# lelecaruso/NavierStokes_Project_NM4PDE

Hardware: AMD Instinct MI355X
Metric: time-steps/sec (assemble_time_step + solve_time_step), 3D flow past a cylinder, P2/P1, Yosida, per-rank ILU(0) (higher is better)
Workload: dtype f64

## Files before the change

### include/nsx.h

```cpp
#ifndef NSX_H
#define NSX_H

#include <stdint.h>

#ifdef __cplusplus
extern "C" {
#endif

typedef struct nsx_handle nsx_handle;

typedef enum {
  NSX_OK = 0,
  NSX_ERR_ARG = -1,
  NSX_ERR_HIP = -2,
  NSX_ERR_UNSUPPORTED = -3,
  NSX_ERR_NOCONV = -4,
  NSX_ERR_NUMERIC = -5,
  NSX_ERR_COMM = -6
} nsx_status;

typedef enum { NSX_PREC_YOSIDA = 0, NSX_PREC_SIMPLE = 1, NSX_PREC_AYOSIDA = 2, NSX_PREC_ASIMPLE = 3 } nsx_prec;

enum {
  NSX_TEMAM = 1,
// ... 168 lines not shown

int nsx_profile_enable(nsx_handle *h, int on);
int nsx_profile_reset(nsx_handle *h);
int nsx_profile_count(nsx_handle *h);
int nsx_profile_get(nsx_handle *h, int i, const char **name, int64_t *launches, double *total_ms, double *bytes_per_launch);

int nsx_persistent_state(nsx_handle *h, int state[4]);

int nsx_path_info(nsx_handle *h, int info[32]);

#define NSX_ILU_FACTOR_LEVEL 1
#define NSX_ILU_FACTOR_LDS 2
#define NSX_ILU_FACTOR_DENSE_ROW 3
#define NSX_ILU_FACTOR_GENERAL 4
#define NSX_ILU_INVERT_NONE 0
#define NSX_ILU_INVERT_LDS 1
#define NSX_ILU_INVERT_GLOBAL 2
#define NSX_ILU_SOLVE_LEVELLED 1
#define NSX_ILU_SOLVE_DENSE 2
#define NSX_ILU_SOLVE_LANES 3
#define NSX_ILU_SOLVE_BLOCK_LDS 4
#define NSX_ILU_SOLVE_BLOCK_GLOBAL 5
int nsx_ilu_path_info(nsx_handle *h, int which, int info[16]);

int nsx_gram_schmidt_cycle(nsx_handle *h, int n, int m, double *vectors, double norm_guard, double *coeffs, double *norms2);
int nsx_gram_schmidt_sweeps(nsx_handle *h, int n, int split, int gap, int m, double *vectors, double norm_guard, int flags, double *coeffs,
                            double *norms2, double *norms2_before, int *normalized);

enum {
  NSX_BLAS1_DOT = 0, NSX_BLAS1_ADD_AND_DOT, NSX_BLAS1_ADD, NSX_BLAS1_ADD_DEV, NSX_BLAS1_SADD, NSX_BLAS1_SCALE, NSX_BLAS1_SCALE_DEV_INV,
  NSX_BLAS1_SCALE_VEC, NSX_BLAS1_AXPY_MULTI, NSX_BLAS1_AXPY_MULTI_INTO, NSX_BLAS1_CG_UPDATE, NSX_BLAS1_CG_DIRECTION, NSX_BLAS1_RECIPROCAL,
  NSX_BLAS1_FINALIZE, NSX_BLAS1_READ, NSX_BLAS1_WRITE_SCALAR, NSX_BLAS1_KIND_COUNT
};
#define NSX_BLAS1_MAX_K 40
typedef struct nsx_blas1_op {
  int32_t kind;
  int32_t d, v, w, x;
  int32_t slot, num, den;
  int32_t count;
  int32_t read;
  int32_t n;
  int32_t k;
  int32_t vs[NSX_BLAS1_MAX_K];
  double a, s;
  double coef[NSX_BLAS1_MAX_K];
} nsx_blas1_op;
// ... 22 lines not shown
```

### navierstokes_project_nm4pde_amd/csrc/nsx_blas.hip

```cpp
#include "nsx_grid.hpp"
#include "nsx_ilu_lanes.hpp"

namespace nsx {

constexpr int RED_BLOCKS = 512;
constexpr int RED_STRIDE = 1024;

struct SRef {
  double c;
  int num, den;
  int num_nb, den_nb;
};

__device__ __forceinline__ double wave_sum_all(double v) {
#pragma unroll
  for (int o = 32; o > 0; o >>= 1) v += __shfl_xor(v, o, 64);
  return v;
}

__device__ __forceinline__ double slot_value(const double *__restrict__ scal, const double *__restrict__ partial, int slot, int nb,
                                             double *sh) {
  if (nb == 0) return scal[slot];
  if (threadIdx.x < 64) {
    const double *p = partial + (size_t)slot * RED_STRIDE;
// ... 505 lines not shown
  if (!h || !info || which < 0 || which > 1) return NSX_ERR_ARG;
  for (int k = 0; k < 16; ++k) info[k] = 0;
  if (!h->have_mesh) return NSX_OK;
  const nsx::IluSchedule &s = which == 0 ? h->schedF : h->schedS;
  const bool stream = s.stream_ncomp > 0 && !s.levelled;
  info[0] = s.path.factor;
  info[1] = s.path.invert;
  info[2] = s.path.solve;
  info[3] = stream ? s.stream_epl : 0;
  info[4] = s.path.solve_pf;
  info[5] = s.path.solve_ncomp;
  info[6] = s.path.solve_f32;
  info[7] = stream ? s.n_waves : 0;
  info[8] = s.n_blocks;
  info[9] = s.max_rows;
  info[10] = s.max_block_nnz;
  info[11] = stream ? s.max_wave_rows : 0;
  info[12] = s.levelled ? 1 : 0;
  info[13] = s.packed_ok ? 1 : 0;
  info[14] = s.dense ? 1 : 0;
  info[15] = s.path.factor_lds_bytes;
  return NSX_OK;
}
```

### navierstokes_project_nm4pde_amd/csrc/nsx_ilu.hip

```cpp
#include <atomic>

#include "nsx_internal.hpp"
#include "nsx_ilu_lanes.hpp"

namespace nsx {

constexpr int ILU_WAVES = 4;
constexpr int ILU_MAXROW = 1024;

__device__ __forceinline__ void pk_store(double *__restrict__ pk_val, float *__restrict__ pk_val32, int sl, double v, int *err) {
  if (pk_val32) {
    const float f = (float)v;
    pk_val32[sl] = f;
    if (!(fabsf(f) <= 3.402823466e+38f)) __hip_atomic_store(err, 5, __ATOMIC_RELAXED, __HIP_MEMORY_SCOPE_SYSTEM);
  } else {
    pk_val[sl] = v;
  }
}

__global__ __launch_bounds__(ILU_WAVES * 64) void k_ilu_factor(const int32_t *__restrict__ bptr, const int32_t *__restrict__ lvl_off,
                                                              const int32_t *__restrict__ lvl_ptr, const int32_t *__restrict__ lvl_rows,
                                                              const int32_t *__restrict__ rp, const int32_t *__restrict__ ci,
                                                              const int32_t *__restrict__ diag, const double *__restrict__ a,
                                                              double *__restrict__ lu, const int32_t *__restrict__ slot_of,
// ... 65 lines not shown
  __shared__ int s_rp[113], s_dg[112];
  const int blk = blockIdx.x, r0 = bptr[blk], n = bptr[blk + 1] - r0;
  const int j = threadIdx.x;
  for (int t = threadIdx.x; t <= n; t += 128) s_rp[t] = rp[r0 + t];
  for (int t = threadIdx.x; t < n; t += 128) s_dg[t] = diag[r0 + t];
  __syncthreads();
  if (j < n) {
    for (int i = 0; i < n; ++i) {
      const int pe = s_dg[i];
      double acc = i == j ? 1.0 : 0.0;
      for (int p = s_rp[i]; p < pe; ++p) {
        const int k = ci[p] - r0;
        if (k >= 0) acc -= lu[p] * Ps[k * n + j];
      }
      Ps[i * n + j] = acc;
    }
    for (int i = n - 1; i >= 0; --i) {
      const int pd = s_dg[i], pe = s_rp[i + 1];
      double acc = lu[pd] * Ps[i * n + j];
      for (int p = pd + 1; p < pe; ++p) {
        const int k = ci[p] - r0;
        if (k < n) acc -= lu[p] * Ps[k * n + j];
      }
      Ps[i * n + j] = acc;
    }
  }
  __syncthreads();
  double *Pb = P + off[blk];
  for (int q = threadIdx.x; q < n * n; q += 128) Pb[q] = Ps[q];
}

__global__ __launch_bounds__(256) void k_ilu_invert(const int32_t *__restrict__ bptr, const int64_t *__restrict__ off,
                                                    const int32_t *__restrict__ rp, const int32_t *__restrict__ ci,
                                                    const int32_t *__restrict__ diag, const double *__restrict__ lu, double *P) {
  const int blk = blockIdx.x, r0 = bptr[blk], n = bptr[blk + 1] - r0;
  double *Pb = P + off[blk];
  for (int j = threadIdx.x; j < n; j += 256) {
    for (int i = 0; i < n; ++i) {
      const int row = r0 + i, pe = diag[row];
      double acc = i == j ? 1.0 : 0.0;
      for (int p = rp[row]; p < pe; ++p) {
        const int k = ci[p] - r0;
        if (k >= 0) acc -= lu[p] * Pb[(size_t)k * n + j];
      }
      Pb[(size_t)i * n + j] = acc;
    }
// ... 371 lines not shown
      s.path.factor = NSX_ILU_FACTOR_LDS;
      s.path.factor_lds_bytes = (int)lds;
      static std::atomic<size_t> lds_allowed{64 * 1024};
      if (lds > lds_allowed.load()) {
        HIP_CHECK(hipFuncSetAttribute((const void *)k_ilu_factor_lds, hipFuncAttributeMaxDynamicSharedMemorySize, 80 * 1024));
        lds_allowed.store(80 * 1024);
      }
      hipLaunchKernelGGL(k_ilu_factor_lds, dim3(s.n_blocks), dim3(ILU_WAVES * 64), lds, h->stream, s.fac_order.p, s.block_ptr.p, s.blk_lvl_off.p, s.fwd_lvl_ptr.p,
                         s.fwd_rows.p, g.rowptr.p, g.colind.p, g.diag.p, s.in_lo.p, s.in_cptr.p, s.in_cpos.p, vals, lu,
                         s.packed_ok ? s.pk_slot_of.p : nullptr, s.pk_val.p, s.pk_dinv.p, err, s.pk_dinv_slot.p, s.max_rows, (int)s.max_block_nnz, pk32);
    } else if (small_ok && s.max_rows <= ILU_DENSE_ROWS) {
      s.path.factor = NSX_ILU_FACTOR_DENSE_ROW;
      hipLaunchKernelGGL(k_ilu_factor_small, dim3(s.n_blocks), dim3(ILU_WAVES * 64), 0, h->stream, s.block_ptr.p, s.blk_lvl_off.p,
                         s.fwd_lvl_ptr.p, s.fwd_rows.p, g.rowptr.p, g.colind.p, g.diag.p, vals, lu, s.packed_ok ? s.pk_slot_of.p : nullptr,
                         s.pk_val.p, s.pk_dinv.p, err, s.pk_dinv_slot.p, pk32);
    } else {
      s.path.factor = NSX_ILU_FACTOR_GENERAL;
      hipLaunchKernelGGL(k_ilu_factor, dim3(s.n_blocks), dim3(ILU_WAVES * 64), 0, h->stream, s.block_ptr.p, s.blk_lvl_off.p, s.fwd_lvl_ptr.p,
                         s.fwd_rows.p, g.rowptr.p, g.colind.p, g.diag.p, vals, lu, s.packed_ok ? s.pk_slot_of.p : nullptr, s.pk_val.p,
                         s.pk_dinv.p, err, s.pk_dinv_slot.p, pk32);
    }
  }
  s.path.invert = NSX_ILU_INVERT_NONE;
  if (s.dense) {
    LaunchScope ls(h, "ilu_invert", 8.0 * (double)s.dn_entries + 12.0 * g.nnz());
    const bool inv_lds = env_on("NSX_ILU_INVERT_LDS");
    const size_t shm = (size_t)s.max_rows * s.max_rows * sizeof(double);
    if (inv_lds && s.max_rows <= 112) {
      static bool attr_set = false;
      if (!attr_set && shm > 64 * 1024) {
        HIP_CHECK(hipFuncSetAttribute((const void *)k_ilu_invert_lds, hipFuncAttributeMaxDynamicSharedMemorySize, 112 * 112 * (int)sizeof(double)));
        attr_set = true;
      }
      s.path.invert = NSX_ILU_INVERT_LDS;
      hipLaunchKernelGGL(k_ilu_invert_lds, dim3(s.n_blocks), dim3(128), shm, h->stream, s.block_ptr.p, s.dn_off.p, g.rowptr.p, g.colind.p, g.diag.p, lu, s.dn_P.p);
    } else {
      s.path.invert = NSX_ILU_INVERT_GLOBAL;
      hipLaunchKernelGGL(k_ilu_invert, dim3(s.n_blocks), dim3(256), 0, h->stream, s.block_ptr.p, s.dn_off.p, g.rowptr.p, g.colind.p, g.diag.p, lu,
                         s.dn_P.p);
    }
  }
}

template <int NCOMP, int LW, bool USE_LDS>
__global__ __launch_bounds__(256) void k_ilu_solve(const int32_t *__restrict__ bptr, const int32_t *__restrict__ offF,
                                                   const int32_t *__restrict__ ptrF, const int32_t *__restrict__ rowsF,
                                                   const int32_t *__restrict__ offB, const int32_t *__restrict__ ptrB,
                                                   const int32_t *__restrict__ rowsB, const int32_t *__restrict__ rp,
                                                   const int32_t *__restrict__ ci, const int32_t *__restrict__ diag,
                                                   const double *__restrict__ lu, const double *__restrict__ b, double *__restrict__ x) {
  extern __shared__ double xs_[];
// ... 284 lines not shown
```

### navierstokes_project_nm4pde_amd/csrc/nsx_internal.hpp

```cpp
#pragma once
#include <hip/hip_runtime.h>

#include <algorithm>
#include <cmath>
#include <cstdint>
#include <cstdio>
#include <cstdlib>
#include <cstring>
#include <exception>
#include <map>
#include <string>
#include <functional>
#include <type_traits>
#include <vector>

#include "../../include/nsx.h"
#include "../host/graph.hpp"

#ifndef NSX_NT
#define NSX_NT 1
#endif
template <int BIT, class T>
__device__ __forceinline__ T ld_stream(const T *p) {
  if constexpr ((NSX_NT & BIT) != 0) return __builtin_nontemporal_load(p);
// ... 101 lines not shown
  int stream_epl = 1;
  int64_t n_slabs = 0;
  int blocks_per_wave = 1, n_waves = 0, max_wave_rows = 0;
  bool packed_ok = false;
  DevBuf<int32_t> pk_row_ptr, pk_rows;
  DevBuf<int32_t> pk_dinv_slot;
  DevBuf<int32_t> pk_slab_ptr;
  DevBuf<int32_t> pk_meta;
  DevBuf<int32_t> pk_slot_of;
  DevBuf<double> pk_val;
  DevBuf<double> pk_dinv;
  DevBuf<float> pk_val32;
  bool stream_f32 = false;
  bool dense = false;
  DevBuf<int64_t> dn_off;
  DevBuf<double> dn_P;
  int64_t dn_entries = 0;
  bool levelled = false;
  std::vector<int32_t> gl_f_ptr_h, gl_b_ptr_h;
  DevBuf<int32_t> gl_f_rows, gl_b_rows, in_lo, in_hi;
  DevBuf<int32_t> gl_f_rec, gl_b_rec;
  struct Path {
    int factor = 0, invert = 0, factor_lds_bytes = 0;
    int solve = 0, solve_pf = 0, solve_ncomp = 0, solve_f32 = 0;
  };
  mutable Path path;
};

inline bool ilu_lanes_stream(const IluSchedule &s, int ncomp) { return s.packed_ok && !s.levelled && !s.dense && s.stream_ncomp == ncomp; }

struct HaloPlan {
  std::vector<int> nbr;
  std::vector<int32_t> send_ptr, recv_ptr;
  std::vector<int32_t> send_idx_in;
  DevBuf<int32_t> send_idx;
  DevBuf<double> sendbuf;
  std::vector<double> h_send, h_recv;
  int n_own = 0;
  hipEvent_t ev_done = nullptr;
  bool in_flight = false;
  bool self_test = false;
};

struct RowSplit {
  DevBuf<int32_t> interior, interface;
  int n_interior = 0, n_interface = 0;
// ... 34 lines not shown
  bool ok = false, values_current = false;
  int64_t n_slots = 0;
  DevBuf<int32_t> u_ptr, u_cols, s_ptr, s_info, s_src;
  DevBuf<uint16_t> s_lidx;
  DevBuf<double> s_val;
  DevBuf<uint16_t> a_lidx;
  int32_t max_block_nnz = 0;
};

struct CgState {
  GridBox box;
  int max_wg = 0;
  int max_wg_res[2] = {0, 0};
  int max_wg_lres[2] = {0, 0};
  bool disabled = false;
  DevBuf<double> vec;
  DevBuf<double> d_vec, d_parts;
  DevBuf<double> d_raw;
  CgPlan plan;
  int d_agreed = -1;
  int last_path = 0;
  int last_rpg = 0, last_lres = 0;
  bool resident = false, lds_resident = false, variant_said = false;
};

struct ProfEntry {
  int64_t launches = 0;
  double bytes = 0;
  double ms = 0;
  std::vector<std::pair<hipEvent_t, hipEvent_t>> pending;
};

struct MgsState {
  GridBox box;
  int max_wg = 0;
  int used_wg[2] = {0, 0}, used_steps[2] = {0, 0};
  int max_wg_e[3] = {0, 0, 0};
  int max_wg_dist[3] = {0, 0, 0};
  int dist_cap_reserved[3] = {0, 0, 0};
  int links = 0;
  bool disabled = false;
  double guard_override = -1.0;
  DevBuf<double> ls_partial, ls_vals, ls_gram;
  int ls_mode = -1;
  DevBuf<double> ext_vals;
  DevBuf<unsigned long long> ext_words;
// ... 247 lines not shown
  nsx::SpmvBlocked blkA;
  int spmv_w = 16;
  bool spmv_blocked = true, spmv_largest_first = true;
  nsx::DevBuf<double> vS0, vMass, vStiff, vConv, vF, vG, vB, vPM, vSchur, luF, luS;
  int inner_precision = NSX_INNER_FP64;
  nsx::DevBuf<float> vF32;
  int inner_F_fp32_used = 0, ilu_F_fp32_used = 0;
  nsx::DevBuf<int32_t> bt_of_g;
  nsx::GatherMap gmA, gmG, gmB, gmPM;
  nsx::DevBuf<double> cellbuf;
  nsx::DevBuf<double> sol, sol_owned, prev_sol, rhs;
  std::vector<int32_t> rank_u_h, rank_p_h, sblk_h;
  nsx::DevBuf<int32_t> rank_u;
  nsx::IluSchedule schedF, schedS;
  nsx::DevBuf<double> dbar;
  nsx::DevBuf<int32_t> bc_dofs;
  nsx::DevBuf<double> bc_vals;
  nsx::DevBuf<double> dirmask;
  std::vector<int32_t> bc_cache;
  nsx::DevBuf<double> diag_D, diag_D_inv, neg_diag_D_inv, lump_M, schur_w;
  nsx::DevBuf<double> schur_w_prev;
  bool schur_valid = false, schur_pending = false;
  int schur_type = -1;
  std::vector<nsx::DevBuf<double> *> pool;
  nsx::DevBuf<double> red_partial;
  nsx::DevBuf<double> scal;
  int slot_nb[nsx::N_SLOTS] = {0};
  double *scal_host = nullptr;
  double *pub_host = nullptr, *pub_dev = nullptr;
  unsigned long long pub_seq = 0;
  nsx::DevBuf<unsigned int> pub_counter;
  nsx::MgsState mgs;
  bool sched_dirty = true;
  int gx_drop_wg = -1;
  int n_persistent_fallbacks = 0;
  int gmres_depth = 0;
  bool cu_reserve_failed = false;
  nsx::DevBuf<double> ext_self;
  hipStream_t stream_plain = nullptr;
  std::vector<hipStream_t> retired_streams;
  int cu_reserved = 0;
  int comm_probe_local = -1;
  long long n_allreduce = 0, n_halo = 0;
  int self_p2p = 0;
  int n_ext_collectives = 0;
  nsx::CgState cg;
// ... 60 lines not shown
  double last;
};
inline int sc_check(int step, double value, double tol, int maxsteps) {
  return value <= tol ? 1 : (step >= maxsteps || std::isnan(value)) ? 2 : 0;
}

inline int env_int(const char *name, int dflt) {
  const char *e = getenv(name);
  return e ? atoi(e) : dflt;
}
inline int64_t env_i64(const char *name, int64_t dflt) {
  const char *e = getenv(name);
  return e ? atoll(e) : dflt;
}
inline double env_double(const char *name, double dflt) {
  const char *e = getenv(name);
  return e ? atof(e) : dflt;
}
inline bool env_set(const char *name) { return getenv(name) != nullptr; }
inline bool env_on(const char *name) { return env_int(name, 1) != 0; }
inline bool env_opt_in(const char *name) { return env_int(name, 0) == 1; }
inline bool nsx_debug() { return env_set("NSX_DEBUG"); }
inline bool ilu_mgs_wanted() { return env_opt_in("NSX_ILU_MGS"); }
inline int ilu_lanes_pf() { return env_int("NSX_PF", 8) == 4 ? 4 : 8; }
inline int mgs_maxwg_cap(int limit) { return env_set("NSX_MGS_MAXWG") ? std::min(limit, env_int("NSX_MGS_MAXWG", 0)) : limit; }

template <int... Vs, class F>
inline bool with_int(int v, F &&f) {
  return ((v == Vs ? (f(std::integral_constant<int, Vs>{}), true) : false) || ...);
}

void setup_ilu_schedule(nsx_handle *h, const Csr &g, const std::vector<int32_t> &block_ptr, IluSchedule &s, int blocks_per_wave, bool allow_dense = false,
                        int ncomp = 1);
void build_schur_graph(nsx_handle *h);
void vec_from_caller(nsx_handle *h, double *dev, const double *host, bool with_ghosts);
void vec_to_caller(nsx_handle *h, const double *dev, double *host);
void part_from_caller(nsx_handle *h, int which, double *dev, const double *host);
void part_to_caller(nsx_handle *h, int which, const double *dev, double *host);
void pressure_from_caller(nsx_handle *h, double *dev, const double *host);
void pressure_to_caller(nsx_handle *h, const double *dev, double *host);
inline int32_t node_to_internal(const nsx_handle *h, int32_t local_node) { return h->layout_on ? h->perm2_h[local_node] : local_node; }
inline int32_t pnode_to_internal(const nsx_handle *h, int32_t local_node) { return h->layout_on ? h->perm1_h[local_node] : local_node; }
void ensure_schedules(nsx_handle *h);

void run_assemble(nsx_handle *h, bool first, int flags);
void run_dirichlet(nsx_handle *h, int n, const int32_t *dofs, const double *vals);

void diag_mesh_setup(nsx_handle *h);
void probe_mesh_setup(nsx_handle *h, const double *cell_coords);
inline void post_mesh_changed(nsx_handle *h) {
  h->probe.mesh_changed();
  h->tracer.mesh_changed();
  h->nodal.mesh_changed();
  h->iso.mesh_changed();
  h->lattice.mesh_changed();
  h->stats.mesh_changed();
  h->surface.mesh_changed();
}

bool blocked_usable(const nsx_handle *h);
void spmv_F(nsx_handle *h, const double *vals, const double *x, double *y, const float *vals32 = nullptr, const double *rb = nullptr);
void spmv_F_inner(nsx_handle *h, const double *x, double *y);
void spmv_F_inner_resid(nsx_handle *h, const double *x, const double *b, double *y);
void convert_F_f32(nsx_handle *h);
void spmv_saddle(nsx_handle *h, const double *x, double *y);
void spmv_G(nsx_handle *h, const double *xp, double *yu, bool accumulate);
void spmv_B(nsx_handle *h, const double *xu, double *yp, const double *r = nullptr, int sub = 0);
void spmv_S(nsx_handle *h, const double *x, double *y);
void schur_numeric(nsx_handle *h, const double *w);
void extract_diag(nsx_handle *h, const DevCsr &g, const double *vals, double *d);
void abs_rowsum(nsx_handle *h, const DevCsr &g, const double *vals, double *d);

void ilu_factor(nsx_handle *h, const DevCsr &g, IluSchedule &s, const double *vals, double *lu, const char *name, bool f32 = false);
void ilu_check(nsx_handle *h);
bool ilu_solve(nsx_handle *h, const DevCsr &g, const IluSchedule &s, const double *lu, const double *b, double *x, int ncomp,
               const char *name, int dot_slot = -1, bool f32 = false, int *used_f32 = nullptr);

struct Span {
  int n, split, gap;
  Span(int n_) : n(n_), split(n_), gap(0) {}
  Span(int n_, int split_, int gap_) : n(n_), split(split_), gap(gap_) {}
};
inline Span blk_span(const nsx_handle *h) { return Span(h->n_u + h->n_p, h->n_u, h->g_u); }

template <int CTRL>
__device__ __forceinline__ double dpp_f64(double v) {
  int lo = __double2loint(v), hi = __double2hiint(v);
  lo = __builtin_amdgcn_update_dpp(0, lo, CTRL, 0xf, 0xf, true);
  hi = __builtin_amdgcn_update_dpp(0, hi, CTRL, 0xf, 0xf, true);
  return __hiloint2double(hi, lo);
}
template <int LW>
// ... 94 lines not shown
```

### navierstokes_project_nm4pde_amd/csrc/nsx_setup.hip

```cpp
#include <algorithm>
#include <cmath>
#include <numeric>

#include "nsx_internal.hpp"
#include "../host/gather_map.hpp"
#include "../host/ilu_levels.hpp"
#include "../host/ilu_stream.hpp"
#include "../host/layout.hpp"
#include "../host/spmv_plan.hpp"

using namespace nsx;

static thread_local std::string g_create_error;

namespace nsx {

static void upload_csr(nsx_handle *h, DevCsr &d, bool square) {
  d.rowptr.upload(d.host.rowptr, h->stream);
  d.colind.upload(d.host.colind, h->stream);
  if (square) {
    std::vector<int32_t> diag(d.host.n_rows);
    for (int32_t i = 0; i < d.host.n_rows; ++i) {
      diag[i] = find_in_row(d.host, i, i);
      if (diag[i] < 0) NSX_THROW(NSX_ERR_ARG, "square graph has no diagonal entry in row %d", i);
// ... 123 lines not shown
  b.n_chunks_if = t.n_chunks_if;
  b.grid_if = t.grid_if;
  b.frac_if = t.frac_if;
  if (b.n_chunks_if) b.desc_if.upload(t.desc_if, h->stream);
  b.crow.upload(bounds, h->stream);
  b.cptr.upload(t.cptr, h->stream);
  b.ucols.upload(t.ucols, h->stream);
  b.lidx.upload(t.lidx, h->stream);
  if (nsx_debug())
    fprintf(stderr, "[nsx] blocked spmv: rows %d chunks %d (max %d rows; %d of them stage a ghost column: %.1f %% of the non-zeros) unique cols/chunk avg %.0f max %d (nnz/unique %.1f)\n",
            g.n_rows, b.n_chunks, b.max_rows, b.n_chunks_if, 100.0 * b.frac_if, b.ucols_total / std::max(1, b.n_chunks), b.max_ucols, (double)g.nnz() / b.ucols_total);
}

static std::vector<int32_t> spmv_chunks(nsx_handle *h) {
  const int target = std::max(16, std::min(448, env_int("NSX_SPMV_R", 130)));
  return chunk_bounds(h->gA.host.n_rows, h->rank_u_h, target, env_on("NSX_SPMV_BY_RANK"));
}

void build_schur_graph(nsx_handle *h) {
  h->gS.host = structural_product(h->gB.host, h->NP, h->NP_loc);
  upload_csr(h, h->gS, true);
  h->vSchur.alloc(h->gS.nnz());
  h->luS.alloc(h->gS.nnz());
}

static void default_ranks(nsx_handle *h) {
  h->in_rank_u_h = {0, h->N2};
  h->in_rank_p_h = {0, h->NP};
  h->in_sblk_h.clear();
}

static void refresh_rank_products(nsx_handle *h) {
  h->rank_u.upload(h->rank_u_h, h->stream);
  h->dbar.alloc(h->rank_u_h.size() - 1);
  h->sched_dirty = true;
  h->prec_ready = false;
  h->schur_valid = false;
  krylov_new_rank_tables(h);
}

void ensure_schedules(nsx_handle *h) {
  if (!h->sched_dirty) return;
  build_blocked(h, h->gA.host, spmv_chunks(h), h->blkA, h->N2);
  auto blocks_per_wave = [](int n_rows, size_t n_blocks) { return std::max(1, std::min(64, (int)(680.0 * (double)n_blocks / std::max(1, n_rows) + 0.5))); };
  const std::vector<int32_t> &sb = h->sblk_h.empty() ? h->rank_p_h : h->sblk_h;
  const int bpwF = env_int("NSX_BPW_F", blocks_per_wave(h->N2, h->rank_u_h.size() - 1));
// ... 848 lines not shown
```

### navierstokes_project_nm4pde_amd/csrc/nsx_sparse.hip

```cpp
#include "nsx_internal.hpp"

namespace nsx {

template <int DIM, int W, bool WITH_G, bool RESID>
__device__ __forceinline__ void spmv_vel_rows(int n_rows, const int32_t *__restrict__ rp, const int32_t *__restrict__ ci,
                                              const double *__restrict__ av, const double *__restrict__ x,
                                              const int32_t *__restrict__ grp, const int32_t *__restrict__ gci,
                                              const double *__restrict__ gv, const double *__restrict__ xp,
                                              double *__restrict__ y, const int32_t *__restrict__ rows, const double *__restrict__ b) {
  const int bid = (blockIdx.x & 7) * (gridDim.x >> 3) + (blockIdx.x >> 3);
  const int slot = (bid * 256 + threadIdx.x) / W, lane = threadIdx.x % W;
  if (slot >= n_rows) return;
  const int row = rows ? rows[slot] : slot;
  double acc[DIM];
#pragma unroll
  for (int c = 0; c < DIM; ++c) acc[c] = 0.0;
  const int e = rp[row + 1];
  for (int p = rp[row] + lane; p < e; p += W) {
    const double a = av[p];
    const double *xj = x + (size_t)ci[p] * DIM;
#pragma unroll
    for (int c = 0; c < DIM; ++c) acc[c] += a * xj[c];
  }
  if (WITH_G) {
// ... 514 lines not shown
  for (int t = threadIdx.x; t < nb; t += 64) {
    const int k = bci[b0 + t];
    rc[t] = k;
#pragma unroll
    for (int c = 0; c < DIM; ++c) rv[t * DIM + c] = bv[(size_t)(b0 + t) * DIM + c] * w[(size_t)k * DIM + c];
  }
  __syncthreads();
  for (int e = srp[i] + threadIdx.x; e < srp[i + 1]; e += 64) {
    const int j = sci[e];
    double acc = 0.0;
    int q = 0;
    for (int p = brp[j]; p < brp[j + 1]; ++p) {
      const int k = bci[p];
      while (q < nb && rc[q] < k) ++q;
      if (q < nb && rc[q] == k) {
#pragma unroll
        for (int c = 0; c < DIM; ++c) acc += rv[q * DIM + c] * bv[(size_t)p * DIM + c];
      }
    }
    sv[e] = acc;
  }
}

void schur_numeric(nsx_handle *h, const double *w) {
  comm_halo_u(h, w);
  int max_row = 0;
  const Csr &B = h->gB.host;
  for (int i = 0; i < B.n_rows; ++i) max_row = std::max(max_row, B.rowptr[i + 1] - B.rowptr[i]);
  const size_t shm = (size_t)max_row * (h->dim * 8 + 4) + 8;
  if (shm > 160 * 1024) NSX_THROW(NSX_ERR_UNSUPPORTED, "row of block(1,0) too long for the Schur kernel (%d)", max_row);
  LaunchScope ls(h, "schur_numeric", 0);
  with_int<2, 3>(h->dim, [&](auto D) {
    hipLaunchKernelGGL((k_schur<decltype(D)::value>), dim3(h->NP), dim3(64), shm, h->stream, h->NP, h->gS.rowptr.p, h->gS.colind.p, h->gB.rowptr.p,
                       h->gB.colind.p, h->vB.p, w, max_row, h->vSchur.p);
  });
}

}
```

### navierstokes_project_nm4pde_amd/nsx.py

```python
import ctypes as C

import numpy as np

from ._lib import DEV_SO, load

_i32p = C.POINTER(C.c_int32)
_f64p = C.POINTER(C.c_double)

TEMAM, DOUBLE_CONVECTION = 1, 2
YOSIDA, SIMPLE, AYOSIDA, ASIMPLE = 0, 1, 2, 3

API = [
    "nsx_create", "nsx_destroy", "nsx_last_error", "nsx_version", "nsx_set_tables", "nsx_set_mesh", "nsx_set_ranks",
    "nsx_set_schur_blocks", "nsx_set_solution", "nsx_get_solution", "nsx_get_solution_ghosted", "nsx_get_rhs",
    "nsx_set_rhs", "nsx_assemble", "nsx_assemble_time_step", "nsx_add_rhs", "nsx_apply_boundary_values",
    "nsx_solve_time_step", "nsx_prec_initialize", "nsx_prec_vmult", "nsx_system_vmult", "nsx_ilu_apply",
    "nsx_export_block", "nsx_schur_nnz", "nsx_schur_get", "nsx_scalar_graph_nnz", "nsx_scalar_graph", "nsx_ilu_get",
    "nsx_profile_enable", "nsx_profile_reset", "nsx_profile_count", "nsx_profile_get", "nsx_persistent_state", "nsx_path_info", "nsx_ilu_path_info", "nsx_comm_self_halo_test", "nsx_comm_unique_id",
    "nsx_comm_init", "nsx_comm_init_callbacks", "nsx_comm_counters", "nsx_set_mesh_distributed", "nsx_set_force_faces", "nsx_compute_forces",
    "nsx_set_internal_layout", "nsx_layout_info", "nsx_layout_get", "nsx_gram_schmidt_cycle", "nsx_set_inner_precision",
    "nsx_gram_schmidt_sweeps", "nsx_compute_diagnostics", "nsx_get_cell_diagnostic", "nsx_schur_cg", "nsx_blas1_run", "nsx_gmres",
    "nsx_set_probes", "nsx_get_probe_cells", "nsx_eval_probes", "nsx_set_tracers", "nsx_advect_tracers", "nsx_get_tracers",
    "nsx_sparse_product", "nsx_compute_nodal_fields", "nsx_nodal_field_components", "nsx_get_nodal_field",
    "nsx_extract_isosurface", "nsx_get_isosurface",
    "nsx_set_lattice", "nsx_get_lattice_cells", "nsx_eval_lattice", "nsx_get_lattice",
    "nsx_stats_begin", "nsx_stats_accumulate", "nsx_stats_info", "nsx_stats_components", "nsx_stats_get",
    "nsx_set_surface", "nsx_surface_info", "nsx_get_surface_layout", "nsx_compute_surface", "nsx_surface_field_components", "nsx_get_surface_field",
]
API_EXTRA = ["nsx_inner_F_vmult"]
FIRST_TOUCH, COLOUR, COLOUR_ALL = 0, 1, 2
INNER_FP64, INNER_FP32 = 0, 1
DIAG_ENERGY, DIAG_DIV2, DIAG_GRAD2, DIAG_ENSTROPHY, DIAG_CHANGE2, DIAG_VOLUME, DIAG_CFL, DIAG_SPEED, DIAG_COUNT = range(9)
PROD_F, PROD_F_INNER, PROD_F_RESID, PROD_MASS, PROD_B, PROD_B_MINUS_R, PROD_R_MINUS_B, PROD_G, PROD_G_ACC, PROD_S, PROD_SADDLE, PROD_COUNT = range(12)
TRACER_EULER, TRACER_RK2, TRACER_RK4 = 1, 2, 4
TRACER_FROZEN, TRACER_LINEAR = 0, 1
TRACER_NOT_FOUND, TRACER_ACTIVE, TRACER_EXITED, TRACER_LOST = 0, 1, 2, 3
FIELD_GRADIENT, FIELD_VORTICITY, FIELD_Q, FIELD_STRAIN, FIELD_DIVERGENCE, FIELD_COUNT = range(6)
ISO_VELOCITY, ISO_PRESSURE, ISO_NODAL, ISO_PLANE = range(4)
LATTICE_VELOCITY, LATTICE_PRESSURE, LATTICE_GRADIENT, LATTICE_NODAL = 1, 2, 4, 8
STATS_VELOCITY, STATS_PRESSURE = 1, 2
(STATS_MEAN_U, STATS_COMOMENT_U, STATS_STRESS_U, STATS_RMS_U, STATS_TKE, STATS_MEAN_P, STATS_COMOMENT_P, STATS_VAR_P, STATS_RMS_P,
# ... 90 lines not shown
    for f in ("nsx_set_solution", "nsx_get_solution", "nsx_get_solution_ghosted", "nsx_get_rhs", "nsx_set_rhs"):
        getattr(L, f).argtypes = [vp, _f64p]
    L.nsx_assemble.argtypes = [vp, C.c_int]
    L.nsx_assemble_time_step.argtypes = [vp, C.c_int]
    L.nsx_add_rhs.argtypes = [vp, C.c_int, _i32p, _f64p]
    L.nsx_apply_boundary_values.argtypes = [vp, C.c_int, _i32p, _f64p]
    L.nsx_solve_time_step.argtypes = [vp, C.c_int, C.c_double, C.c_double, C.c_int, C.c_int, C.POINTER(Stats)]
    L.nsx_prec_initialize.argtypes = [vp, C.c_int]
    L.nsx_prec_vmult.argtypes = [vp, C.c_int, C.c_double, C.c_int, _f64p, _f64p, C.POINTER(Stats)]
    L.nsx_system_vmult.argtypes = [vp, _f64p, _f64p]
    L.nsx_ilu_apply.argtypes = [vp, C.c_int, _f64p, _f64p]
    L.nsx_export_block.argtypes = [vp, C.c_int, C.c_int, C.c_int, _i32p, _i32p, _f64p]
    L.nsx_schur_nnz.argtypes = [vp, C.POINTER(C.c_int64)]
    L.nsx_schur_get.argtypes = [vp, _i32p, _i32p, _f64p]
    L.nsx_scalar_graph_nnz.argtypes = [vp, C.c_int, C.POINTER(C.c_int64)]
    L.nsx_scalar_graph.argtypes = [vp, C.c_int, _i32p, _i32p]
    L.nsx_ilu_get.argtypes = [vp, C.c_int, _f64p]
    L.nsx_profile_enable.argtypes = [vp, C.c_int]
    L.nsx_profile_reset.argtypes = [vp]
    L.nsx_profile_count.argtypes = [vp]
    L.nsx_profile_get.argtypes = [vp, C.c_int, C.POINTER(C.c_char_p), C.POINTER(C.c_int64), _f64p, _f64p]
    L.nsx_persistent_state.argtypes = [vp, C.POINTER(C.c_int)]
    L.nsx_ilu_path_info.argtypes = [vp, C.c_int, C.POINTER(C.c_int)]
    L.nsx_comm_unique_id.argtypes = [C.POINTER(C.c_uint8)]
    L.nsx_comm_init.argtypes = [vp, C.c_int, C.c_int, C.POINTER(C.c_uint8)]
    L.nsx_comm_init_callbacks.argtypes = [vp, C.c_int, C.c_int, ALLREDUCE_FN, EXCHANGE_FN, C.c_void_p]
    L.nsx_comm_counters.argtypes = [vp, C.POINTER(C.c_longlong)]
    L.nsx_set_mesh_distributed.argtypes = [vp, C.c_int, C.c_int, C.c_int, _i32p, _f64p, C.c_int, C.c_int, C.c_int, C.c_int,
                                           _i32p, _i32p, C.c_int, _i32p, _i32p, _i32p, _i32p, _i32p]
    L.nsx_set_force_faces.argtypes = [vp, C.c_int, _i32p, _i32p, C.c_int, _f64p, _f64p, _f64p, _f64p]
    L.nsx_compute_forces.argtypes = [vp, _f64p, _f64p]
    L.nsx_compute_diagnostics.argtypes = [vp, C.POINTER(FlowDiag)]
    L.nsx_get_cell_diagnostic.argtypes = [vp, C.c_int, _f64p]
    L.nsx_set_probes.argtypes = [vp, C.c_int, _f64p, C.c_double]
    L.nsx_get_probe_cells.argtypes = [vp, _i32p, _i32p, _f64p]
    L.nsx_eval_probes.argtypes = [vp, _f64p, _f64p, _f64p, _i32p]
    L.nsx_set_tracers.argtypes = [vp, C.c_int, _f64p, C.c_double]
    L.nsx_advect_tracers.argtypes = [vp, C.c_double, C.c_int, C.c_int, C.c_int]
    L.nsx_get_tracers.argtypes = [vp, _f64p, _i32p, _i32p, _i32p, _f64p]
    L.nsx_compute_nodal_fields.argtypes = [vp]
    L.nsx_nodal_field_components.argtypes = [vp, C.c_int, C.POINTER(C.c_int)]
    L.nsx_get_nodal_field.argtypes = [vp, C.c_int, _f64p]
    L.nsx_extract_isosurface.argtypes = [vp, C.POINTER(IsoSource), C.c_double, C.POINTER(IsoSource), C.POINTER(C.c_int64)]
    L.nsx_get_isosurface.argtypes = [vp, _f64p, _f64p, _i32p]
    L.nsx_set_lattice.argtypes = [vp, _f64p, _f64p, _i32p, C.c_double, C.POINTER(C.c_int64)]
    L.nsx_get_lattice_cells.argtypes = [vp, _i32p]
# ... 121 lines not shown
                 "schur_dense_inverses", "sweep_off", "fallbacks", "rccl_sweep_velocity_plain", "rccl_sweep_velocity_masked", "rccl_sweep_block_plain",
                 "rccl_sweep_block_masked", "schur_blocks_per_partial", "sweep_velocity_one_gpu", "owned_p2_nodes", "owned_p1_nodes", "sweep_with_ilu_inside", "fused_launches",
                 "inner_F_fp32", "ilu_F_fp32", "schur_cg_rows_per_lane_group", "schur_cg_operator_in_lds",
                 "spmv_max_chunk_rows", "spmv_max_staged_columns")

    def path_info(self):
        v = (C.c_int * 32)()
        self._ck(self.L.nsx_path_info(self._h, v))
        return {k: int(v[i]) for i, k in enumerate(self.PATH_KEYS)}

    ILU_PATH_KEYS = ("factor", "invert", "solve", "entries_per_tick", "slabs_per_set", "ncomp", "float_stream", "waves", "blocks", "max_block_rows",
                     "max_block_nnz", "max_wave_rows", "levelled", "lane_stream", "dense_inverses", "factor_lds_bytes")
    ILU_FACTOR = {0: None, 1: "level", 2: "lds", 3: "dense_row", 4: "general"}
    ILU_INVERT = {0: None, 1: "lds", 2: "global"}
    ILU_SOLVE = {0: None, 1: "levelled", 2: "dense", 3: "lanes", 4: "block_lds", 5: "block_global"}

    def ilu_path_info(self, which):
        v = (C.c_int * 16)()
        self._ck(self.L.nsx_ilu_path_info(self._h, int(which), v))
        d = {k: int(v[i]) for i, k in enumerate(self.ILU_PATH_KEYS)}
        d["factor"], d["invert"], d["solve"] = self.ILU_FACTOR[d["factor"]], self.ILU_INVERT[d["invert"]], self.ILU_SOLVE[d["solve"]]
        return d

    def comm_counters(self):
        c = (C.c_longlong * 2)()
        self._ck(self.L.nsx_comm_counters(self._h, c))
        return int(c[0]), int(c[1])

    def comm_self_halo_test(self, n_own, n_ghost, ncomp):
        e = C.c_double(0.0)
        self._ck(self.L.nsx_comm_self_halo_test(self._h, int(n_own), int(n_ghost), int(ncomp), C.byref(e)))
        return float(e.value)

    def comm_init_single(self):
        ident = (C.c_uint8 * 128)()
        self._ck(self.L.nsx_comm_unique_id(ident))
        self._ck(self.L.nsx_comm_init(self._h, 0, 1, ident))

    def gather_solution(self):
        x = np.zeros(self.n)
        self._ck(self.L.nsx_get_solution(self._h, _d(x)))
        if self.world > 1:
            import torch
            import torch.distributed as dist
            t = torch.from_numpy(x)
            if dist.get_backend() == "nccl":
# ... 432 lines not shown
```

Measured before the change: 14.31.

## Precompute Schur product pair plan and stage ILU factor rows in LDS for inversion

Adds a host-built plan that lists, for each entry of the Schur complement S = B W B^T, the matching pairs of block(1,0) entries. The numeric Schur kernel then runs over the precomputed pairs with a gather, replacing the per-entry sorted merge of two B rows. Separately, when LDS inversion is enabled, a new invert kernel stages each block's L/U values and 16-bit column indices in shared memory before the dense triangular inversion. The plan costs extra device memory (capped by NSX_SCHUR_PLAN_MB) and setup time, and the staged inversion needs more LDS per block.

After: 14.49 (median of 6 runs). 1.01x the previous value.

```diff
diff --git a/include/nsx.h b/include/nsx.h
--- a/include/nsx.h
+++ b/include/nsx.h
@@ -214,6 +214,10 @@
 #define NSX_ILU_SOLVE_BLOCK_LDS 4
 #define NSX_ILU_SOLVE_BLOCK_GLOBAL 5
 int nsx_ilu_path_info(nsx_handle *h, int which, int info[16]);
+
+#define NSX_SCHUR_PRODUCT_MERGE 1
+#define NSX_SCHUR_PRODUCT_PLANNED 2
+int nsx_schur_setup_info(nsx_handle *h, int64_t info[8]);
 
 int nsx_gram_schmidt_cycle(nsx_handle *h, int n, int m, double *vectors, double norm_guard, double *coeffs, double *norms2);
 int nsx_gram_schmidt_sweeps(nsx_handle *h, int n, int split, int gap, int m, double *vectors, double norm_guard, int flags, double *coeffs,
diff --git a/navierstokes_project_nm4pde_amd/csrc/nsx_blas.hip b/navierstokes_project_nm4pde_amd/csrc/nsx_blas.hip
--- a/navierstokes_project_nm4pde_amd/csrc/nsx_blas.hip
+++ b/navierstokes_project_nm4pde_amd/csrc/nsx_blas.hip
@@ -551,3 +551,18 @@
   info[15] = s.path.factor_lds_bytes;
   return NSX_OK;
 }
+
+extern "C" int nsx_schur_setup_info(nsx_handle *h, int64_t info[8]) {
+  if (!h || !info) return NSX_ERR_ARG;
+  for (int k = 0; k < 8; ++k) info[k] = 0;
+  if (!h->have_mesh) return NSX_OK;
+  const nsx::SchurSetup &ss = h->schur_setup;
+  info[0] = ss.last_product;
+  info[1] = ss.plan_status;
+  info[2] = ss.n_pairs;
+  info[3] = ss.n_walked;
+  info[4] = ss.bytes;
+  info[5] = h->schedS.path.invert_staged;
+  info[6] = ss.max_row;
+  return NSX_OK;
+}
diff --git a/navierstokes_project_nm4pde_amd/csrc/nsx_ilu.hip b/navierstokes_project_nm4pde_amd/csrc/nsx_ilu.hip
--- a/navierstokes_project_nm4pde_amd/csrc/nsx_ilu.hip
+++ b/navierstokes_project_nm4pde_amd/csrc/nsx_ilu.hip
@@ -111,6 +111,54 @@
         const int k = ci[p] - r0;
         if (k < n) acc -= lu[p] * Ps[k * n + j];
       }
+      Ps[i * n + j] = acc;
+    }
+  }
+  __syncthreads();
+  double *Pb = P + off[blk];
+  for (int q = threadIdx.x; q < n * n; q += 128) Pb[q] = Ps[q];
+}
+
+__host__ __device__ inline size_t ilu_invert_staged_bytes(int max_rows, int max_nz) {
+  const size_t nz = ((size_t)max_nz + 3) & ~(size_t)3;
+  return (size_t)max_rows * max_rows * 8 + nz * 10 + (size_t)(max_rows + 4) * 2 * 2;
+}
+__global__ __launch_bounds__(128) void k_ilu_invert_staged(const int32_t *__restrict__ bptr, const int64_t *__restrict__ off,
+                                                           const int32_t *__restrict__ ci, const int32_t *__restrict__ diag,
+                                                           const int32_t *__restrict__ in_lo, const int32_t *__restrict__ cptr,
+                                                           const int32_t *__restrict__ cpos, const double *__restrict__ lu,
+                                                           double *__restrict__ P, int max_rows, int max_nz) {
+  extern __shared__ double Ps[];
+  const int nzp = (max_nz + 3) & ~3, mr = max_rows + 4;
+  double *fv = Ps + (size_t)max_rows * max_rows;
+  uint16_t *fc = (uint16_t *)(fv + nzp);
+  uint16_t *frp = fc + nzp;
+  uint16_t *fdg = frp + mr;
+  const int blk = blockIdx.x, r0 = bptr[blk], n = bptr[blk + 1] - r0;
+  const int j = threadIdx.x;
+  const int c0 = cptr[r0], nzb = cptr[r0 + n] - c0;
+  for (int t = threadIdx.x; t <= n; t += 128) frp[t] = (uint16_t)(cptr[r0 + t] - c0);
+  for (int t = threadIdx.x; t < n; t += 128) fdg[t] = (uint16_t)(cptr[r0 + t] - c0 + diag[r0 + t] - in_lo[r0 + t]);
+#pragma unroll 4
+  for (int e = threadIdx.x; e < nzb; e += 128) {
+    const int p = cpos[c0 + e];
+    fv[e] = lu[p];
+    fc[e] = (uint16_t)(ci[p] - r0);
+  }
+  __syncthreads();
+  if (j < n) {
+    for (int i = 0; i < n; ++i) {
+      const int pe = fdg[i];
+      double acc = i == j ? 1.0 : 0.0;
+#pragma unroll 4
+      for (int e = frp[i]; e < pe; ++e) acc -= fv[e] * Ps[fc[e] * n + j];
+      Ps[i * n + j] = acc;
+    }
+    for (int i = n - 1; i >= 0; --i) {
+      const int pd = fdg[i], pe = frp[i + 1];
+      double acc = fv[pd] * Ps[i * n + j];
+#pragma unroll 4
+      for (int e = pd + 1; e < pe; ++e) acc -= fv[e] * Ps[fc[e] * n + j];
       Ps[i * n + j] = acc;
     }
   }
@@ -528,11 +576,23 @@
     }
   }
   s.path.invert = NSX_ILU_INVERT_NONE;
+  s.path.invert_staged = 0;
   if (s.dense) {
     LaunchScope ls(h, "ilu_invert", 8.0 * (double)s.dn_entries + 12.0 * g.nnz());
     const bool inv_lds = env_on("NSX_ILU_INVERT_LDS");
     const size_t shm = (size_t)s.max_rows * s.max_rows * sizeof(double);
-    if (inv_lds && s.max_rows <= 112) {
+    const size_t shm_staged = ilu_invert_staged_bytes(s.max_rows, s.max_block_nnz);
+    if (inv_lds && s.max_rows <= 112 && s.max_block_nnz < 65535 && shm_staged <= 160 * 1024 && !schur_setup_legacy()) {
+      static std::atomic<size_t> staged_allowed{64 * 1024};
+      if (shm_staged > staged_allowed.load()) {
+        HIP_CHECK(hipFuncSetAttribute((const void *)k_ilu_invert_staged, hipFuncAttributeMaxDynamicSharedMemorySize, (int)shm_staged));
+        staged_allowed.store(shm_staged);
+      }
+      s.path.invert = NSX_ILU_INVERT_LDS;
+      s.path.invert_staged = 1;
+      hipLaunchKernelGGL(k_ilu_invert_staged, dim3(s.n_blocks), dim3(128), shm_staged, h->stream, s.block_ptr.p, s.dn_off.p, g.colind.p, g.diag.p, s.in_lo.p,
+                         s.in_cptr.p, s.in_cpos.p, lu, s.dn_P.p, s.max_rows, (int)s.max_block_nnz);
+    } else if (inv_lds && s.max_rows <= 112) {
       static bool attr_set = false;
       if (!attr_set && shm > 64 * 1024) {
         HIP_CHECK(hipFuncSetAttribute((const void *)k_ilu_invert_lds, hipFuncAttributeMaxDynamicSharedMemorySize, 112 * 112 * (int)sizeof(double)));
diff --git a/navierstokes_project_nm4pde_amd/csrc/nsx_internal.hpp b/navierstokes_project_nm4pde_amd/csrc/nsx_internal.hpp
--- a/navierstokes_project_nm4pde_amd/csrc/nsx_internal.hpp
+++ b/navierstokes_project_nm4pde_amd/csrc/nsx_internal.hpp
@@ -147,6 +147,7 @@
   DevBuf<int32_t> gl_f_rec, gl_b_rec;
   struct Path {
     int factor = 0, invert = 0, factor_lds_bytes = 0;
+    int invert_staged = 0;
     int solve = 0, solve_pf = 0, solve_ncomp = 0, solve_f32 = 0;
   };
   mutable Path path;
@@ -227,6 +228,15 @@
   int last_path = 0;
   int last_rpg = 0, last_lres = 0;
   bool resident = false, lds_resident = false, variant_said = false;
+};
+
+struct SchurSetup {
+  DevBuf<int32_t> ptr;
+  DevBuf<uint32_t> pair;
+  int plan_status = -1;
+  int64_t n_pairs = 0, n_walked = 0, bytes = 0;
+  int max_row = 0;
+  int last_product = 0;
 };
 
 struct ProfEntry {
@@ -520,6 +530,7 @@
   nsx::DevBuf<double> schur_w_prev;
   bool schur_valid = false, schur_pending = false;
   int schur_type = -1;
+  nsx::SchurSetup schur_setup;
   std::vector<nsx::DevBuf<double> *> pool;
   nsx::DevBuf<double> red_partial;
   nsx::DevBuf<double> scal;
@@ -626,6 +637,10 @@
 inline bool env_opt_in(const char *name) { return env_int(name, 0) == 1; }
 inline bool nsx_debug() { return env_set("NSX_DEBUG"); }
 inline bool ilu_mgs_wanted() { return env_opt_in("NSX_ILU_MGS"); }
+inline bool schur_setup_legacy() {
+  const char *e = getenv("NSX_SCHUR_SETUP");
+  return e && !strcmp(e, "legacy");
+}
 inline int ilu_lanes_pf() { return env_int("NSX_PF", 8) == 4 ? 4 : 8; }
 inline int mgs_maxwg_cap(int limit) { return env_set("NSX_MGS_MAXWG") ? std::min(limit, env_int("NSX_MGS_MAXWG", 0)) : limit; }
 
@@ -672,6 +687,7 @@
 void spmv_B(nsx_handle *h, const double *xu, double *yp, const double *r = nullptr, int sub = 0);
 void spmv_S(nsx_handle *h, const double *x, double *y);
 void schur_numeric(nsx_handle *h, const double *w);
+void build_schur_product_plan(nsx_handle *h);
 void extract_diag(nsx_handle *h, const DevCsr &g, const double *vals, double *d);
 void abs_rowsum(nsx_handle *h, const DevCsr &g, const double *vals, double *d);
 
diff --git a/navierstokes_project_nm4pde_amd/csrc/nsx_setup.hip b/navierstokes_project_nm4pde_amd/csrc/nsx_setup.hip
--- a/navierstokes_project_nm4pde_amd/csrc/nsx_setup.hip
+++ b/navierstokes_project_nm4pde_amd/csrc/nsx_setup.hip
@@ -169,6 +169,7 @@
   upload_csr(h, h->gS, true);
   h->vSchur.alloc(h->gS.nnz());
   h->luS.alloc(h->gS.nnz());
+  build_schur_product_plan(h);
 }
 
 static void default_ranks(nsx_handle *h) {
diff --git a/navierstokes_project_nm4pde_amd/csrc/nsx_sparse.hip b/navierstokes_project_nm4pde_amd/csrc/nsx_sparse.hip
--- a/navierstokes_project_nm4pde_amd/csrc/nsx_sparse.hip
+++ b/navierstokes_project_nm4pde_amd/csrc/nsx_sparse.hip
@@ -1,4 +1,5 @@
 #include "nsx_internal.hpp"
+#include "../host/schur_plan.hpp"
 
 namespace nsx {
 
@@ -560,17 +561,93 @@
   }
 }
 
+template <int DIM>
+__global__ __launch_bounds__(64) void k_schur_planned(int n_rows, const int32_t *__restrict__ srp, const int32_t *__restrict__ sci,
+                                                      const int32_t *__restrict__ brp, const int32_t *__restrict__ bci,
+                                                      const double *__restrict__ bv, const double *__restrict__ w,
+                                                      const int32_t *__restrict__ pptr, const uint32_t *__restrict__ pair,
+                                                      double *__restrict__ sv) {
+  extern __shared__ double smem[];
+  double *rv = smem;
+  const int i = blockIdx.x;
+  if (i >= n_rows) return;
+  const int b0 = brp[i], nb = brp[i + 1] - b0;
+  for (int t = threadIdx.x; t < nb; t += 64) {
+    const int k = bci[b0 + t];
+#pragma unroll
+    for (int c = 0; c < DIM; ++c) rv[t * DIM + c] = bv[(size_t)(b0 + t) * DIM + c] * w[(size_t)k * DIM + c];
+  }
+  __syncthreads();
+  constexpr int U = 4;
+  for (int e = srp[i] + threadIdx.x; e < srp[i + 1]; e += 64) {
+    const double *bj = bv + (size_t)brp[sci[e]] * DIM;
+    const int t0 = pptr[e], t1 = pptr[e + 1];
+    double acc = 0.0;
+    for (int t = t0; t < t1; t += U) {
+      uint32_t u[U];
+      double b[U][DIM];
+#pragma unroll
+      for (int s = 0; s < U; ++s) u[s] = pair[t + s < t1 ? t + s : t];
+#pragma unroll
+      for (int s = 0; s < U; ++s)
+#pragma unroll
+        for (int c = 0; c < DIM; ++c) b[s][c] = bj[(size_t)(u[s] & 0xffffu) * DIM + c];
+#pragma unroll
+      for (int s = 0; s < U; ++s) {
+        double a = acc;
+#pragma unroll
+        for (int c = 0; c < DIM; ++c) a += rv[(u[s] >> 16) * DIM + c] * b[s][c];
+        acc = t + s < t1 ? a : acc;
+      }
+    }
+    sv[e] = acc;
+  }
+}
+
+void build_schur_product_plan(nsx_handle *h) {
+  SchurSetup &ss = h->schur_setup;
+  const Csr &B = h->gB.host;
+  ss.max_row = 0;
+  for (int i = 0; i < B.n_rows; ++i) ss.max_row = std::max(ss.max_row, B.rowptr[i + 1] - B.rowptr[i]);
+  const int64_t cap_bytes = env_i64("NSX_SCHUR_PLAN_MB", 512) << 20;
+  const int64_t fixed = 4 * (h->gS.nnz() + 1);
+  const SchurPlan pl = build_schur_plan(B, h->gS.host, std::max<int64_t>(0, (cap_bytes - fixed) / 4));
+  ss.plan_status = pl.status;
+  ss.n_pairs = pl.n_pairs;
+  ss.n_walked = pl.n_walked;
+  ss.bytes = 0;
+  ss.last_product = 0;
+  ss.ptr.release();
+  ss.pair.release();
+  if (pl.status == SCHUR_PLAN_NOT_IN_PATTERN) NSX_THROW(NSX_ERR_ARG, "internal: the Schur pattern is not the structural product of block(1,0)");
+  if (pl.status == SCHUR_PLAN_OK) {
+    ss.ptr.upload(pl.ptr, h->stream);
+    ss.pair.upload(pl.pair, h->stream);
+    ss.bytes = fixed + 4 * pl.n_pairs;
+  }
+  if (nsx_debug())
+    fprintf(stderr, "[nsx] schur product: %lld entries, %lld pairs (the merge without a plan walks %lld entries of block(1,0), longest row %d)%s, plan %.1f MB\n",
+            (long long)h->gS.nnz(), (long long)ss.n_pairs, (long long)ss.n_walked, ss.max_row,
+            pl.status == SCHUR_PLAN_OK ? "" : pl.status == SCHUR_PLAN_TOO_LARGE ? ": above NSX_SCHUR_PLAN_MB, no plan (k_schur)" : ": a row above 65535 entries, no plan (k_schur)",
+            1e-6 * (double)ss.bytes);
+}
+
 void schur_numeric(nsx_handle *h, const double *w) {
   comm_halo_u(h, w);
-  int max_row = 0;
-  const Csr &B = h->gB.host;
-  for (int i = 0; i < B.n_rows; ++i) max_row = std::max(max_row, B.rowptr[i + 1] - B.rowptr[i]);
-  const size_t shm = (size_t)max_row * (h->dim * 8 + 4) + 8;
+  SchurSetup &ss = h->schur_setup;
+  const int max_row = ss.max_row;
+  const bool planned = ss.plan_status == SCHUR_PLAN_OK && !schur_setup_legacy();
+  const size_t shm = (size_t)max_row * (h->dim * 8 + (planned ? 0 : 4)) + 8;
   if (shm > 160 * 1024) NSX_THROW(NSX_ERR_UNSUPPORTED, "row of block(1,0) too long for the Schur kernel (%d)", max_row);
   LaunchScope ls(h, "schur_numeric", 0);
+  ss.last_product = planned ? NSX_SCHUR_PRODUCT_PLANNED : NSX_SCHUR_PRODUCT_MERGE;
   with_int<2, 3>(h->dim, [&](auto D) {
-    hipLaunchKernelGGL((k_schur<decltype(D)::value>), dim3(h->NP), dim3(64), shm, h->stream, h->NP, h->gS.rowptr.p, h->gS.colind.p, h->gB.rowptr.p,
-                       h->gB.colind.p, h->vB.p, w, max_row, h->vSchur.p);
+    if (planned)
+      hipLaunchKernelGGL((k_schur_planned<decltype(D)::value>), dim3(h->NP), dim3(64), shm, h->stream, h->NP, h->gS.rowptr.p, h->gS.colind.p, h->gB.rowptr.p,
+                         h->gB.colind.p, h->vB.p, w, ss.ptr.p, ss.pair.p, h->vSchur.p);
+    else
+      hipLaunchKernelGGL((k_schur<decltype(D)::value>), dim3(h->NP), dim3(64), shm, h->stream, h->NP, h->gS.rowptr.p, h->gS.colind.p, h->gB.rowptr.p,
+                         h->gB.colind.p, h->vB.p, w, max_row, h->vSchur.p);
   });
 }
 
diff --git a/navierstokes_project_nm4pde_amd/host/schur_plan.hpp b/navierstokes_project_nm4pde_amd/host/schur_plan.hpp
--- /dev/null
+++ b/navierstokes_project_nm4pde_amd/host/schur_plan.hpp
@@ -0,0 +1,74 @@
+#pragma once
+#include <cstdint>
+#include <vector>
+
+#include "graph.hpp"
+
+namespace nsx {
+
+enum { SCHUR_PLAN_OK = 0, SCHUR_PLAN_TOO_LARGE = 1, SCHUR_PLAN_ROW_TOO_LONG = 2, SCHUR_PLAN_NOT_IN_PATTERN = 3 };
+
+struct SchurPlan {
+  int status = SCHUR_PLAN_OK;
+  std::vector<int32_t> ptr;
+  std::vector<uint32_t> pair;
+  int64_t n_pairs = 0;
+  int64_t n_walked = 0;
+};
+
+inline SchurPlan build_schur_plan(const Csr &B, const Csr &S, int64_t max_pairs) {
+  SchurPlan pl;
+  const int32_t n = S.n_rows;
+  for (int64_t e = 0; e < S.nnz(); ++e) pl.n_walked += B.rowptr[S.colind[e] + 1] - B.rowptr[S.colind[e]];
+  std::vector<int32_t> tptr((size_t)B.n_cols + 1, 0), trow((size_t)B.nnz()), tpos((size_t)B.nnz());
+  for (int64_t p = 0; p < B.nnz(); ++p) tptr[B.colind[p] + 1]++;
+  for (int32_t k = 0; k < B.n_cols; ++k) tptr[k + 1] += tptr[k];
+  {
+    std::vector<int32_t> fill(tptr.begin(), tptr.end() - 1);
+    for (int32_t j = 0; j < B.n_rows; ++j)
+      for (int32_t p = B.rowptr[j]; p < B.rowptr[j + 1]; ++p) {
+        const int32_t t = fill[B.colind[p]]++;
+        trow[t] = j;
+        tpos[t] = p - B.rowptr[j];
+      }
+  }
+  for (int32_t i = 0; i < n; ++i)
+    for (int32_t kb = B.rowptr[i]; kb < B.rowptr[i + 1]; ++kb) pl.n_pairs += tptr[B.colind[kb] + 1] - tptr[B.colind[kb]];
+  for (int32_t j = 0; j < B.n_rows; ++j)
+    if (B.rowptr[j + 1] - B.rowptr[j] > 65535) pl.status = SCHUR_PLAN_ROW_TOO_LONG;
+  if (pl.status == SCHUR_PLAN_OK && (pl.n_pairs > max_pairs || pl.n_pairs > INT32_MAX)) pl.status = SCHUR_PLAN_TOO_LARGE;
+  if (pl.status != SCHUR_PLAN_OK) return pl;
+  std::vector<int32_t> entry_of((size_t)S.n_cols, -1), cursor;
+  pl.ptr.assign((size_t)S.nnz() + 1, 0);
+  for (int pass = 0; pass < 2 && pl.status == SCHUR_PLAN_OK; ++pass) {
+    if (pass == 1) {
+      for (int64_t e = 0; e < S.nnz(); ++e) pl.ptr[e + 1] += pl.ptr[e];
+      cursor.assign(pl.ptr.begin(), pl.ptr.end() - 1);
+      pl.pair.resize((size_t)pl.n_pairs);
+    }
+    for (int32_t i = 0; i < n && pl.status == SCHUR_PLAN_OK; ++i) {
+      for (int32_t e = S.rowptr[i]; e < S.rowptr[i + 1]; ++e) entry_of[S.colind[e]] = e;
+      for (int32_t kb = B.rowptr[i]; kb < B.rowptr[i + 1]; ++kb) {
+        const int32_t k = B.colind[kb];
+        const uint32_t q = (uint32_t)(kb - B.rowptr[i]) << 16;
+        for (int32_t t = tptr[k]; t < tptr[k + 1]; ++t) {
+          const int32_t e = trow[t] < S.n_cols ? entry_of[trow[t]] : -1;
+          if (e < 0) {
+            pl.status = SCHUR_PLAN_NOT_IN_PATTERN;
+            break;
+          }
+          if (pass == 0) pl.ptr[e + 1]++;
+          else pl.pair[cursor[e]++] = q | (uint32_t)tpos[t];
+        }
+      }
+      for (int32_t e = S.rowptr[i]; e < S.rowptr[i + 1]; ++e) entry_of[S.colind[e]] = -1;
+    }
+  }
+  if (pl.status != SCHUR_PLAN_OK) {
+    pl.ptr.clear();
+    pl.pair.clear();
+  }
+  return pl;
+}
+
+}
diff --git a/navierstokes_project_nm4pde_amd/nsx.py b/navierstokes_project_nm4pde_amd/nsx.py
--- a/navierstokes_project_nm4pde_amd/nsx.py
+++ b/navierstokes_project_nm4pde_amd/nsx.py
@@ -16,7 +16,7 @@
     "nsx_set_rhs", "nsx_assemble", "nsx_assemble_time_step", "nsx_add_rhs", "nsx_apply_boundary_values",
     "nsx_solve_time_step", "nsx_prec_initialize", "nsx_prec_vmult", "nsx_system_vmult", "nsx_ilu_apply",
     "nsx_export_block", "nsx_schur_nnz", "nsx_schur_get", "nsx_scalar_graph_nnz", "nsx_scalar_graph", "nsx_ilu_get",
-    "nsx_profile_enable", "nsx_profile_reset", "nsx_profile_count", "nsx_profile_get", "nsx_persistent_state", "nsx_path_info", "nsx_ilu_path_info", "nsx_comm_self_halo_test", "nsx_comm_unique_id",
+    "nsx_profile_enable", "nsx_profile_reset", "nsx_profile_count", "nsx_profile_get", "nsx_persistent_state", "nsx_path_info", "nsx_ilu_path_info", "nsx_schur_setup_info", "nsx_comm_self_halo_test", "nsx_comm_unique_id",
     "nsx_comm_init", "nsx_comm_init_callbacks", "nsx_comm_counters", "nsx_set_mesh_distributed", "nsx_set_force_faces", "nsx_compute_forces",
     "nsx_set_internal_layout", "nsx_layout_info", "nsx_layout_get", "nsx_gram_schmidt_cycle", "nsx_set_inner_precision",
     "nsx_gram_schmidt_sweeps", "nsx_compute_diagnostics", "nsx_get_cell_diagnostic", "nsx_schur_cg", "nsx_blas1_run", "nsx_gmres",
@@ -153,6 +153,7 @@
     L.nsx_profile_get.argtypes = [vp, C.c_int, C.POINTER(C.c_char_p), C.POINTER(C.c_int64), _f64p, _f64p]
     L.nsx_persistent_state.argtypes = [vp, C.POINTER(C.c_int)]
     L.nsx_ilu_path_info.argtypes = [vp, C.c_int, C.POINTER(C.c_int)]
+    L.nsx_schur_setup_info.argtypes = [vp, C.POINTER(C.c_int64)]
     L.nsx_comm_unique_id.argtypes = [C.POINTER(C.c_uint8)]
     L.nsx_comm_init.argtypes = [vp, C.c_int, C.c_int, C.POINTER(C.c_uint8)]
     L.nsx_comm_init_callbacks.argtypes = [vp, C.c_int, C.c_int, ALLREDUCE_FN, EXCHANGE_FN, C.c_void_p]
@@ -320,6 +321,17 @@
         d["factor"], d["invert"], d["solve"] = self.ILU_FACTOR[d["factor"]], self.ILU_INVERT[d["invert"]], self.ILU_SOLVE[d["solve"]]
         return d
 
+    SCHUR_SETUP_KEYS = ("product", "no_plan", "pairs", "walked_without_plan", "plan_bytes", "invert_factor_in_lds", "longest_row_of_B")
+    SCHUR_PRODUCT = {0: None, 1: "merge", 2: "planned"}
+    SCHUR_NO_PLAN = {0: None, 1: "above NSX_SCHUR_PLAN_MB", 2: "a row above 65535 entries"}
+
+    def schur_setup_info(self):
+        v = (C.c_int64 * 8)()
+        self._ck(self.L.nsx_schur_setup_info(self._h, v))
+        d = {k: int(v[i]) for i, k in enumerate(self.SCHUR_SETUP_KEYS)}
+        d["product"], d["no_plan"] = self.SCHUR_PRODUCT[d["product"]], self.SCHUR_NO_PLAN[d["no_plan"]]
+        return d
+
     def comm_counters(self):
         c = (C.c_longlong * 2)()
         self._ck(self.L.nsx_comm_counters(self._h, c))
```
